# his0si/ConvNet-Quantization

Hardware: AMD Instinct MI355X
Metric: images/sec at batch 1024 (3×32×32) int8 static-PTQ, 1/2/4/8 MI355X; top-1 delta (higher is better)
Workload: dtype int8; 1 GPU; full static-PTQ SimpleConvNet, all conv+linear int8 (u8 x s8 -> i32), NHWC, per-tensor weights; global_batch=1024, per_gpu_batch=1024, parallelism=dp1

## Files before the change

### convnet-quantization_amd/csrc/conv3x3.hip

```cpp
#include "common.hpp"
#include "conv_epi.hpp"
#include "conv_launch.hpp"
#include <type_traits>
#include <utility>
#include <algorithm>
#include <cmath>
#include "qconvnet_abi.hpp"

namespace qcn {

constexpr int kPipeD = 2;
constexpr int kSm56D = 4;
constexpr int kProdPrio = 2;

template <int CIN, int COUT, int HW, bool POOL, int WPX, int PSP = 16, int RPAD = 0,
          int SPAD = 0, bool SPLIT = false, int WI_ = 2, int JT_ = 4, int RB_ = 0>
struct ConvCfg {
  static constexpr int kCin = CIN, kCout = COUT;
  static constexpr bool kPool = POOL, kSplit = SPLIT;
  static constexpr int W = HW, H = HW;
  static constexpr int WI = WI_;
  static constexpr int JT = JT_;
  static constexpr int MPS = JT * WI;
  static constexpr int kWpx = WPX;
// ... 1320 lines not shown
      return dst ? reinterpret_cast<float4*>(eka) + e : const_cast<float4*>(reinterpret_cast<const float4*>(s) + o);
    }
    e -= NA;
    if (e < NB) {
      const int a = e / (CB::kCout / 4), o = e % (CB::kCout / 4);
      const float* s = a == 0 ? epb.u : (a == 1 ? epb.v : epb.mult);
      return dst ? reinterpret_cast<float4*>(ekb) + e : const_cast<float4*>(reinterpret_cast<const float4*>(s) + o);
    }
    e -= NB;
    if (e < NCA)
      return dst ? reinterpret_cast<float4*>(cra) + e
                 : const_cast<float4*>(reinterpret_cast<const float4*>(epa.corr) + e);
    e -= NCA;
    return dst ? reinterpret_cast<float4*>(crb) + e
               : const_cast<float4*>(reinterpret_cast<const float4*>(epb.corr) + e);
  };
  {
    const uint32_t pa4 = xor80(splat_u8(x_zp)), pb4 = xor80(splat_u8(xb_zp));
    auto halo = [&](auto cfg, uint8_t* base, int nbuf, int pbytes, uint32_t pad) {
      using C = decltype(cfg);
      constexpr int HS = 2 * C::PCOLS + 2 * (C::PROWS - 2), CH = C::kCin / 16;
      const int total = nbuf * C::SEGS * HS * CH;
      for (int e = tid; e < total; e += 512) {
        const int c = e % CH, hs = (e / CH) % HS, sg = (e / (CH * HS)) % C::SEGS, bf = e / (CH * HS * C::SEGS);
        int pr, pc;
        if (hs < C::PCOLS) { pr = 0; pc = hs; }
        else if (hs < 2 * C::PCOLS) { pr = C::PROWS - 1; pc = hs - C::PCOLS; }
        else { const int r = hs - 2 * C::PCOLS; pr = 1 + (r >> 1); pc = (r & 1) ? C::PCOLS - 1 : 0; }
        *reinterpret_cast<uint4*>(base + bf * pbytes + C::slot(sg, pr, pc) + c * 16) = make_uint4(pad, pad, pad, pad);
      }
    };
    halo(CA{}, lds + P::OFF_PA, P::DOUBLE_A ? 2 : 1, P::PA, pa4);
    halo(CB{}, lds + P::OFF_PB, 2, P::PB, pb4);
  }
  if (role == 1) {
#pragma unroll
    for (int k = 0; k < TPT; ++k)
      if (rt + 256 * k < NTAB) tval[k] = *tab(rt + 256 * k, false);
#pragma unroll
    for (int k = 0; k < TPT; ++k)
      if (rt + 256 * k < NTAB) *tab(rt + 256 * k, true) = tval[k];
  }
  if (T == 0) return;

  const int p16 = lane & 15, g = lane >> 4;
  const wt_rsrc_t wra = wt_rsrc(wa), wrb = wt_rsrc(wb);
  const int voff = (wc * 64 + p16) * 64 + g * 16;
  auto pa_buf = [&](int j) { return lds + P::OFF_PA + (P::DOUBLE_A ? (j & 1) * P::PA : 0); };
  auto pb_buf = [&](int j) { return lds + P::OFF_PB + (j & 1) * P::PB; };
  auto write_in = [&](uint8_t* pa, const uint4 (&sv)[4]) {
#pragma unroll
    for (int q = 0; q < 4; ++q)
      *reinterpret_cast<uint4*>(pa + in_dst(q)) =
          make_uint4(xor80(sv[q].x), xor80(sv[q].y), xor80(sv[q].z), xor80(sv[q].w));
  };
  auto first_chunk = [&](wt_rsrc_t w0, v4i (&ga)[2][4]) {
#pragma unroll
    for (int i = 0; i < 4; ++i) {
      const auto v = __builtin_amdgcn_raw_buffer_load_b128(w0, voff, i * 1024, 0);
      ga[0][i] = (v4i){(int)v[0], (int)v[1], (int)v[2], (int)v[3]};
    }
  };

  v4i acc[4][8];
  if (role == 0) write_in(pa_buf(0), sv0);
  lds_barrier();

  struct Lane {
    int p16, g, ek;
    int la, lb;
    int hb;
    int q;
    const int *ca, *cb;
  };
  auto lanes = [&]() {
    int lz = lane;
    asm volatile("" : "+v"(lz));
    Lane L;
    L.p16 = lz & 15;
    L.g = lz >> 4;
    L.ek = wc * 64 + 4 * L.g;
    L.la = XA::at(wp, 0, L.p16) + 16 * L.g;
    L.lb = XB::at(wp, 0, L.p16) + 16 * L.g;
    L.hb = XA::template out_at<CB>(wp, 0, L.p16) + wc * 64 + 4 * L.g;
    L.q = wp * 32 + L.p16;
    L.ca = cra + (lz >> 6);
    L.cb = crb + (lz >> 6);
    return L;
  };
  auto epi_a = [&](const Lane& L, uint8_t* pb) {
    static_for<4>([&](auto ic) {
      constexpr int i = decltype(ic)::value;
      const EpiG K = load_epig(eka, CA::kCout, L.ek + 16 * i);
      static_for<8>([&](auto jc) {
        constexpr int j = decltype(jc)::value;
        uint32_t wd = 0;
#pragma unroll
        for (int r = 0; r < 4; ++r) wd = rq_elem<FA>(acc[i][j][r], K, r, epa, wd);
        *reinterpret_cast<uint32_t*>(pb + L.hb + XA::template out_jofs<CB>(j) + 16 * i) = xor80(wd);
      });
    });
  };
  auto epi_b = [&](const Lane& L, int k) {
    static_for<2>([&](auto gc) {
      constexpr int gq = decltype(gc)::value;
      uint32_t d[4];
      static_for<4>([&](auto ic) {
        constexpr int i = decltype(ic)::value;
        const EpiG K = load_epig(ekb, CB::kCout, L.ek + 16 * i);
        uint32_t wd = 0;
#pragma unroll
        for (int r = 0; r < 4; ++r) {
          const int a = max(max(acc[i][4 * gq][r], acc[i][4 * gq + 1][r]),
                            max(acc[i][4 * gq + 2][r], acc[i][4 * gq + 3][r]));
          wd = rq_elem<FB>(a, K, r, epb, wd);
        }
        d[i] = wd;
      });
      const auto s02 = __builtin_amdgcn_permlane32_swap(d[0], d[2], false, false);
      const auto s13 = __builtin_amdgcn_permlane32_swap(d[1], d[3], false, false);
      const auto t01 = __builtin_amdgcn_permlane16_swap(s02[0], s13[0], false, false);
      const auto t23 = __builtin_amdgcn_permlane16_swap(s02[1], s13[1], false, false);
      const uint4 v = make_uint4(t01[0], t01[1], t23[0], t23[1]);
      const int q = L.q + 16 * gq;
      const int n = img_of(k, q / P::OPI), pix = q % P::OPI;
      const int co = wc * 64 + 16 * L.g;
      const bool real = ILV ? b + (k * SEGS + q / P::OPI) * G < nimg : (b + k * G) * SEGS + q / P::OPI < nimg;
      if (real) {
        if constexpr (KMAJOR) {
          const int kc = (pix * CB::kCout + co) / 32;
          store_wt16(wt_rsrc(y), (uint32_t)(((long)kc * nimg + n) * 32 + 16 * (L.g & 1)), v);
        } else {
          store_wt16(wt_rsrc(y + (long)n * P::OPI * CB::kCout), (uint32_t)(pix * CB::kCout + co), v);
        }
      }
    });
  };

  if (role == 0) {
    v4i ga[2][4];
    first_chunk(wra, ga);
    uint4 sv[4] = {};
#pragma unroll 1
    for (int p = 0; p <= T; ++p) {
      if constexpr (!P::DOUBLE_A) {
        if (p >= 1 && p < T) write_in(pa_buf(p), sv);
        lds_barrier();
      }
      WS16_STAMP(p, 0);
      if (p < T) {
        const Lane L = lanes();
        pipe_job16<CA>(pa_buf(p), L.ca, wra, wra, voff, wc, L.la, L.g, acc, ga);
        WS16_STAMP(p, 1);
        const int kn = p + 1 < T ? p + 1 : p;
#pragma unroll
        for (int q = 0; q < 4; ++q) sv[q] = *reinterpret_cast<const uint4*>(in_src(kn, q));
        epi_a(L, pb_buf(p));
        if constexpr (P::DOUBLE_A) write_in(pa_buf(p + 1), sv);
        WS16_STAMP(p, 2);
      }
      lds_barrier();
    }
  } else {
    v4i ga[2][4];
    first_chunk(wrb, ga);
#pragma unroll 1
    for (int p = 0; p <= T; ++p) {
      if constexpr (!P::DOUBLE_A) lds_barrier();
      WS16_STAMP(p, 0);
      if (p >= 1) {
        const Lane L = lanes();
        if (p >= 2) epi_b(L, p - 2);
        WS16_STAMP(p, 1);
        pipe_job16<CB>(pb_buf(p - 1), L.cb, wrb, wrb, voff, wc, L.lb, L.g, acc, ga);
        WS16_STAMP(p, 2);
      }
      lds_barrier();
    }
    const Lane L = lanes();
    epi_b(L, T - 1);
#ifdef QCN_CONVNET_STAMP
    if (T + 1 < 8) { WS16_STAMP(T + 1, 0); }
#endif
  }
}

template <class CA, class CB, int FA, int FB, bool KMAJOR>
__global__ __launch_bounds__(512, 1)
void convpair_ws16_kernel(const uint8_t* __restrict__ x, int nimg, int x_zp, const int8_t* __restrict__ wa,
                          ConvEpi epa, int xb_zp, const int8_t* __restrict__ wb, ConvEpi epb,
                          uint8_t* __restrict__ y) {
  convpair_ws16_body<CA, CB, FA, FB, KMAJOR>((int)blockIdx.x, (int)gridDim.x, x, nimg, x_zp, wa, epa, xb_zp,
                                             wb, epb, y);
}

using W16A3 = ConvCfg<64, 128, 16, false, 2, 32, 0, 0, false>;
using W16B4 = ConvCfg<128, 128, 16, true, 2, 32, 64, 0, true>;
using W16A5 = ConvCfg<128, 256, 8, false, 1, 32, 192, 0, false>;
using W16B6 = ConvCfg<256, 256, 8, true, 1, 32, 0, 0, true>;

struct Conv1Cfg {
  static constexpr int H = 32, W = 32, R = 16, COUT = 64, NT = 256;
  static constexpr int PXB = R * W;
  static constexpr int PR = R + 2, PC = W + 2;
  static constexpr int PATCH = 3 * PR * PC;
  static constexpr int PATCH_AL = (PATCH + 15) / 16 * 16;
  static constexpr int KS = 32 + 16;
  static constexpr int LDS = PATCH_AL + PXB * KS;
};

template <int HW>
__global__ __launch_bounds__(256, 3)
void conv1_f32_kernel(const float* __restrict__ x, int nimg, float in_inv, int in_zp,
                      const int8_t* __restrict__ w1, ConvEpi ep, uint8_t* __restrict__ y,
                      uint8_t* __restrict__ qin_out) {
  constexpr int H = HW, W = HW;
  constexpr int R = (HW * HW >= 512) ? 512 / W : H;
  constexpr int SEGS = (HW * HW >= 512) ? 1 : 512 / (HW * HW);
  constexpr int PR = R + 2, PC = W + 2;
  constexpr int PATCH = SEGS * 3 * PR * PC;
  constexpr int PATCH_AL = (PATCH + 15) / 16 * 16;
  constexpr int KS = 48;
  extern __shared__ __attribute__((aligned(16))) uint8_t lds[];
  int8_t* patch = reinterpret_cast<int8_t*>(lds);
  uint8_t* cols = lds + PATCH_AL;

  const int tid = threadIdx.x, lane = tid & 63, wave = tid >> 6;
  const int l32 = lane & 31, hi = lane >> 5;
  const long p0 = (long)blockIdx.x * 512;
  const int n0 = (int)(p0 / (H * W));
  const int y0 = (int)((p0 % (H * W)) / W);
  const int8_t padv = (int8_t)(in_zp - 128);

  for (int it = tid; it < PATCH; it += 256) {
    const int seg = it / (3 * PR * PC);
    const int rem = it % (3 * PR * PC);
    const int c = rem / (PR * PC);
    const int rr = (rem / PC) % PR, cc = rem % PC;
    const int n = n0 + seg, yy = y0 + rr - 1, xx = cc - 1;
    int8_t v = padv;
    if (n < nimg && yy >= 0 && yy < H && xx >= 0 && xx < W) {
      const long gi = (((long)n * 3 + c) * H + yy) * W + xx;
      float t = x[gi] * in_inv;
      t = fminf(fmaxf(t, -1.0e9f), 1.0e9f);
      int q = (int)__builtin_rintf(t) + in_zp;
      q = q < 0 ? 0 : (q > 255 ? 255 : q);
      v = (int8_t)(q - 128);
      if (qin_out != nullptr && seg < SEGS && rr >= 1 && rr <= R && cc >= 1 && cc <= W)
        qin_out[(((long)n * H + yy) * W + xx) * 3 + c] = (uint8_t)q;
    }
    patch[it] = v;
  }
  __syncthreads();
  for (int pp = tid; pp < 512; pp += 256) {
    const int seg = pp / (R * W), yy = (pp / W) % R, xx = pp % W;
    uint32_t wds[8];
#pragma unroll
    for (int d = 0; d < 8; ++d) {
      uint32_t wv = 0;
#pragma unroll
      for (int bb = 0; bb < 4; ++bb) {
        const int k = d * 4 + bb;
        uint32_t byte = 0;
        if (k < 27) {
          const int tap = k / 3, c = k % 3, r = tap / 3, s = tap % 3;
          byte = (uint8_t)patch[((seg * 3 + c) * PR + yy + r) * PC + xx + s];
        }
        wv |= byte << (8 * bb);
      }
      wds[d] = wv;
    }
    uint4* dst = reinterpret_cast<uint4*>(cols + pp * KS);
    dst[0] = make_uint4(wds[0], wds[1], wds[2], wds[3]);
    dst[1] = make_uint4(wds[4], wds[5], wds[6], wds[7]);
  }
  __syncthreads();

  v4i a[2];
#pragma unroll
  for (int i = 0; i < 2; ++i)
    a[i] = *reinterpret_cast<const v4i*>(w1 + (i * 32 + l32) * 32 + hi * 16);
  v16i acc[2][4];
#pragma unroll
  for (int j = 0; j < 4; ++j) {
    const int m = (wave * 4 + j) * 32 + l32;
    const v4i b = *reinterpret_cast<const v4i*>(cols + m * KS + hi * 16);
#pragma unroll
    for (int i = 0; i < 2; ++i)
      acc[i][j] = __builtin_amdgcn_mfma_i32_32x32x32_i8(a[i], b, acc_init_corr(ep.corr, i * 32, hi),
                                                        0, 0, 0);
  }
  __syncthreads();
  uint8_t* lout = lds;
#pragma unroll
  for (int i = 0; i < 2; ++i)
#pragma unroll
    for (int j = 0; j < 4; ++j)
      epilogue_tile<1>(&acc[i][j], ep, i * 32, hi, lout + ((wave * 4 + j) * 32 + l32) * 80);
  __syncthreads();
  const long total = (long)nimg * H * W;
  store_staged<64, 80, 256>(lout, 512, y + p0 * 64, total - p0, tid);
}

using Conv2Cfg = ConvCfg<64, 64, 32, true, 4, 16, 96, 0, true>;

struct Conv12P {
  using C = Conv2Cfg;
  static constexpr int PATCH = C::PATCH;
  static constexpr int WRES = 9 * C::WBUF;
  static constexpr int IN_R = 20, IN_C = 40;
  static constexpr int IN8 = IN_R * IN_C * 4;
  static constexpr int OFF_W = 2 * PATCH;
  static constexpr int OFF_IN = OFF_W + WRES;
  static constexpr int OFF_EPI1 = OFF_IN + 2 * IN8;
  static constexpr int OFF_EPI2 = OFF_EPI1 + 12 * 64;
  static constexpr int OFF_CORR2 = OFF_EPI2 + 12 * 64;
  static constexpr int OFF_A1 = OFF_CORR2 + 4 * 64;
  static constexpr int OFF_CORR1 = OFF_A1 + 2 * 64 * 16;
  static constexpr int LDS = OFF_CORR1 + 4 * 64;
  static_assert(LDS <= 160 * 1024, "LDS budget");
  static constexpr int OFF_QLUT = LDS;
  static constexpr int LDS_U8 = OFF_QLUT + 3 * 256;
  static_assert(OFF_QLUT % 4 == 0 && LDS_U8 <= 160 * 1024, "LDS budget");
};

template <class C>
QCN_DEV void conv_mainloop_res(const uint8_t* patch, const uint8_t* wres,
                               const int* __restrict__ corr, int wave, int lane,
                               v16i (&acc)[2][4]) {
  constexpr int CB = C::kCin / 64;
  const int wc = wave % C::WCO, wp = wave / C::WCO;
  const int l32 = lane & 31, hi = lane >> 5;
  const PatchAddr<C> pa(wp, l32, hi);
  const int arow = wc * 64 + l32;
  const int aswz = (arow >> 2) & 3;
  v16i c0[2];
#pragma unroll
  for (int i = 0; i < 2; ++i) c0[i] = acc_init_corr(corr, wc * 64 + i * 32, hi);
  const uint8_t* abase = wres + arow * 64;
  auto rd_a = [&](int ch, int kk, int i) {
    return *reinterpret_cast<const v4i*>(abase + ch * C::WBUF + i * 32 * 64 +
                                         (((2 * kk + hi) ^ aswz) << 4));
  };
  auto rd_b = [&](int ch, int kk, int j) {
    const int tap = ch / CB, cb = ch % CB;
    return *reinterpret_cast<const v4i*>(patch + pa.base[j] + PatchAddr<C>::delta(tap, j) + cb * 64 +
                                         kk * 32);
  };
  auto step = [&](v4i (&fan)[2], v4i (&fbn)[4], int rch, int rkk, bool rd,
                  const v4i (&fa)[2], const v4i (&fb)[4], bool first) {
#pragma unroll
    for (int m = 0; m < 8; ++m) {
      if (rd) {
        if (m < 2) fan[m] = rd_a(rch, rkk, m);
        else if (m < 6) fbn[m - 2] = rd_b(rch, rkk, m - 2);
      }
      __builtin_amdgcn_sched_barrier(0);
      acc[m >> 2][m & 3] = __builtin_amdgcn_mfma_i32_32x32x32_i8(
          fa[m >> 2], fb[m & 3], first ? c0[m >> 2] : acc[m >> 2][m & 3], 0, 0, 0);
      __builtin_amdgcn_sched_barrier(0);
    }
  };
  v4i fa0[2], fb0[4], fa1[2], fb1[4];
  fa0[0] = rd_a(0, 0, 0);
  fa0[1] = rd_a(0, 0, 1);
#pragma unroll
  for (int j = 0; j < 4; ++j) fb0[j] = rd_b(0, 0, j);
#pragma unroll
  for (int ch = 0; ch < C::NCH; ++ch) {
    step(fa1, fb1, ch, 1, true, fa0, fb0, ch == 0);
    step(fa0, fb0, ch + 1, 0, ch + 1 < C::NCH, fa1, fb1, false);
  }
}

#ifdef QCN_C12_STAMP
__device__ unsigned long long g_c12_stamp[4096][3][12][3];
QCN_DEV void c12_stamp(int j, int k) {
  const unsigned long long t = __builtin_amdgcn_s_memtime();
  const unsigned lane = __builtin_amdgcn_mbcnt_hi(~0u, __builtin_amdgcn_mbcnt_lo(~0u, 0u));
  const int w = threadIdx.x >> 6;
  const int s = w == 0 ? 0 : (w == 4 ? 1 : (w == 5 ? 2 : -1));
  if (s >= 0 && lane == 0 && blockIdx.x < 4096 && j < 12) {
    volatile unsigned long long* d = &g_c12_stamp[blockIdx.x][s][j][k];
    *d = t + lane;
  }
}
#define C12_STAMP(j, k) c12_stamp(j, k)
#else
#define C12_STAMP(j, k)
#endif

template <class XT>
QCN_DEV void conv12p_body(int t0, int ts, int T, const XT* __restrict__ x, int nimg,
                          float in_inv, int in_zp, const int8_t* __restrict__ w1, ConvEpi ep1,
                          int x2_zp, const int8_t* __restrict__ w2, ConvEpi ep2,
                          uint8_t* __restrict__ y, const uint8_t* __restrict__ qlut = nullptr) {
  using C = Conv2Cfg;
  using L = Conv12P;
  constexpr bool U8 = std::is_same<XT, uint8_t>::value;
  static_assert(U8 || std::is_same<XT, float>::value, "fp32 NCHW or u8 NHWC input");
  extern __shared__ __attribute__((aligned(16))) uint8_t lds[];
  const int tid = threadIdx.x, lane = tid & 63, wave = tid >> 6;
  const bool producer = wave >= 4;
  const int ptid = tid - 320;
  auto tile_of = [&](int j) { return (t0 + (j >> 1) * ts) * 2 + (j & 1); };
  uint8_t* patch0 = lds;
  uint8_t* patch1 = lds + L::PATCH;
  uint8_t* in8_0 = lds + L::OFF_IN;
  uint8_t* in8_1 = lds + L::OFF_IN + L::IN8;

  typename std::conditional<U8, uint32_t, float4>::type xraw[3];
  const uint32_t padw = xor80(splat_u8(x2_zp));
  const uint4 pad4 = make_uint4(padw, padw, padw, padw);
  for (int e = tid; e < 2 * C::PROWS * 8; e += 512) {
    const int buf = e / (C::PROWS * 8), r = e % (C::PROWS * 8);
    const int pr = r / 8, pc = ((r / 4) & 1) ? C::PCOLS - 1 : 0, chunk = r & 3;
    *reinterpret_cast<uint4*>(lds + buf * L::PATCH + C::slot(0, pr, pc) + chunk * 16) = pad4;
  }

  auto setup = [&]() {
    if (!producer) {
      const int wave_u = __builtin_amdgcn_readfirstlane(wave);
#pragma unroll
      for (int i = 0; i < L::WRES / 4096; ++i) {
        const int p = i * 4 + wave_u;
        const int o = p * 1024 + lane * 16;
        const int ch = o / C::WBUF, oc = o % C::WBUF;
        const int r = oc >> 6, sl = (oc >> 4) & 3;
        glds16(w2 + (long)ch * C::WBUF + r * 64 + ((sl ^ ((r >> 2) & 3)) << 4), lds + L::OFF_W + p * 1024);
      }
    }

    const uint32_t in_pad = xor80(splat_u8(in_zp)) & 0x00ffffffu;
    for (int e = tid; e < 2 * L::IN_R * L::IN_C; e += 512) {
      const int b = e / (L::IN_R * L::IN_C), rc = e % (L::IN_R * L::IN_C);
      const int rr = rc / L::IN_C, cc = rc % L::IN_C;
      const bool pad_row = b == 0 ? rr < 2 : rr >= 18;
      if (pad_row || cc < 4 || cc >= 36)
        reinterpret_cast<uint32_t*>(lds + L::OFF_IN + b * L::IN8)[rc] = in_pad;
    }
    if (!producer) stage_epik<64, 256>(ep1, reinterpret_cast<float*>(lds + L::OFF_EPI1), tid);
    if (!producer) stage_epik<64, 256>(ep2, reinterpret_cast<float*>(lds + L::OFF_EPI2), tid);
    {
      int t = tid;
      asm volatile("" : "+v"(t));
      if (t < 16)
        reinterpret_cast<int4*>(lds + L::OFF_CORR2)[t] = reinterpret_cast<const int4*>(ep2.corr)[t];
      if (t >= 64 && t < 80)
        reinterpret_cast<int4*>(lds + L::OFF_CORR1)[t - 64] = reinterpret_cast<const int4*>(ep1.corr)[t - 64];
    }
    if (wave == 3) {
      const int l32 = lane & 31, hi = lane >> 5;
      v4i* a1t = reinterpret_cast<v4i*>(lds + L::OFF_A1);
#pragma unroll
      for (int i = 0; i < 2; ++i) {
        const uint4 r0 = *reinterpret_cast<const uint4*>(w1 + (i * 32 + l32) * 32);
        const uint4 r1 = *reinterpret_cast<const uint4*>(w1 + (i * 32 + l32) * 32 + 16);
        const uint32_t wd[8] = {r0.x, r0.y, r0.z, r0.w, r1.x, r1.y, r1.z, r1.w};
        auto byte = [&](int k) -> uint32_t { return (wd[k >> 2] >> (8 * (k & 3))) & 0xff; };
        auto tapw = [&](int t) -> int {
          return (int)(byte(3 * t) | (byte(3 * t + 1) << 8) | (byte(3 * t + 2) << 16));
        };
        const v4i lo4 = (v4i){tapw(0) | (int)(byte(24) << 24), tapw(1) | (int)(byte(25) << 24),
                              tapw(2) | (int)(byte(26) << 24), tapw(3)};
        const v4i hi4 = (v4i){tapw(4), tapw(5), tapw(6), tapw(7)};
        a1t[i * 64 + lane] = hi ? hi4 : lo4;
      }
    }
    if constexpr (U8) {
      for (int e = tid; e < 3 * 256; e += 512) lds[L::OFF_QLUT + e] = qlut[e] ^ 0x80;
    }
  };
  auto fresh_ptid = [&]() {
    int v = ptid;
    asm volatile("" : "+v"(v));
    return v;
  };
  auto stage_load = [&](int t) {
    if (ptid < 0) return;
    const int n = t >> 1, y0 = (t & 1) * 16;
    const int pt = fresh_ptid();
    const int r = pt < 144 ? pt >> 3 : 0, g = pt & 7;
    const int iy = y0 + (y0 == 0 ? 0 : -2) + r;
    const int nc = n < nimg ? n : nimg - 1;
    if constexpr (U8) {
      const uint32_t* p = reinterpret_cast<const uint32_t*>(x + (((long)nc * 32 + iy) * 32 + 4 * g) * 3);
#pragma unroll
      for (int c = 0; c < 3; ++c) xraw[c] = p[c];
    } else {
#pragma unroll
      for (int c = 0; c < 3; ++c)
        xraw[c] = *reinterpret_cast<const float4*>(x + (((long)nc * 3 + c) * 32 + iy) * 32 + 4 * g);
    }
  };
  auto stage_store = [&](uint8_t* in8, int half) {
    const int pt = fresh_ptid();
    if (pt >= 0 && pt < 144) {
      const int rr = (half ? 0 : 2) + (pt >> 3), g = pt & 7;
      uint32_t wd[4];
      if constexpr (U8) {
        const uint8_t* lut = lds + L::OFF_QLUT;
#pragma unroll
        for (int e = 0; e < 4; ++e) {
          uint32_t d = 0;
#pragma unroll
          for (int c = 0; c < 3; ++c) {
            const int k = 3 * e + c;
            const uint32_t b = (xraw[k >> 2] >> (8 * (k & 3))) & 0xffu;
            d |= (uint32_t)lut[c * 256 + b] << (8 * c);
          }
          wd[e] = d;
        }
      } else {
        const float zpf = (float)in_zp;
#pragma unroll
        for (int e = 0; e < 4; ++e) {
          uint32_t d = 0;
#pragma unroll
          for (int c = 0; c < 3; ++c) {
            const float xv = e == 0 ? xraw[c].x : e == 1 ? xraw[c].y : e == 2 ? xraw[c].z : xraw[c].w;
            d = __builtin_amdgcn_cvt_pk_u8_f32(__builtin_rintf(xv * in_inv) + zpf, c, d);
          }
          wd[e] = d ^ 0x00808080u;
        }
      }
      *reinterpret_cast<uint4*>(in8 + (rr * L::IN_C + 4 + 4 * g) * 4) = make_uint4(wd[0], wd[1], wd[2], wd[3]);
    }
  };
  auto fresh = [](int v) {
    asm volatile("" : "+v"(v));
    return v;
  };
  bool vuni = false, muni = false;
  const bool fast1 = epi_fast(ep1);
  auto conv1_tile = [&](int t, const uint8_t* in8, uint8_t* pb, const uint8_t* prev, int w,
                        int step) {
    __builtin_amdgcn_s_setprio(kProdPrio);
    const int h = t & 1, y0 = h * 16;
    const int r0 = h == 0 ? 1 : (prev ? 2 : 0), r1 = h == 0 ? 18 : 17;
    const int ln = fresh(lane), l32 = ln & 31, hi = ln >> 5;
    if (w == step - 1) {
      uint8_t* prow_ptr = pb + C::slot(0, h == 0 ? 0 : 17, l32 + 1);
      *reinterpret_cast<uint4*>(prow_ptr + hi * 32) = pad4;
      *reinterpret_cast<uint4*>(prow_ptr + hi * 32 + 16) = pad4;
    }
    if (prev) {
      for (int e = w * 64 + ln; e < 2 * C::RS / 16; e += step * 64)
        *reinterpret_cast<uint4*>(pb + C::slot(0, 0, 0) + e * 16) =
            *reinterpret_cast<const uint4*>(prev + C::slot(0, 16, 0) + e * 16);
    }
    const float* ek1 = reinterpret_cast<const float*>(lds + L::OFF_EPI1);
    v4i a1[2];
    v16i c1[2];
    {
      const v4i* a1t = reinterpret_cast<const v4i*>(lds + L::OFF_A1);
      const int* corr1 = reinterpret_cast<const int*>(lds + L::OFF_CORR1);
#pragma unroll
      for (int i = 0; i < 2; ++i) {
        a1[i] = a1t[i * 64 + ln];
        c1[i] = acc_init_corr(corr1, i * 32, hi);
      }
    }
    const int* in32 = reinterpret_cast<const int*>(in8);
    auto bop = [&](int tr, v4i& b0) {
      const int* r0 = in32 + (tr + 0) * L::IN_C + l32 + 3;
      const int* r1 = r0 + L::IN_C;
      const int* r2 = r1 + L::IN_C;
      if (hi == 0) {
        const uint32_t t8 = (uint32_t)r2[2];
        b0 = (v4i){(int)__builtin_amdgcn_perm((uint32_t)r0[0], t8, 0x00060504u),
                   (int)__builtin_amdgcn_perm((uint32_t)r0[1], t8, 0x01060504u),
                   (int)__builtin_amdgcn_perm((uint32_t)r0[2], t8, 0x02060504u), r1[0]};
      } else {
        b0 = (v4i){r1[1], r1[2], r2[0], r2[1]};
      }
    };
    auto rows = [&](auto mode) {
      constexpr int MODE = decltype(mode)::value > 2 ? decltype(mode)::value - 2 : decltype(mode)::value;
      constexpr bool AFF = decltype(mode)::value > 2;
      float u[2][16], m[2][16];
      const float sv = ek1[64], sm = ek1[128];
      if constexpr (MODE != 0) {
#pragma unroll
        for (int i = 0; i < 2; ++i)
#pragma unroll
          for (int g = 0; g < 4; ++g) {
            const int co = i * 32 + 8 * g + 4 * hi;
            const float4 u4 = *reinterpret_cast<const float4*>(ek1 + co);
            u[i][4 * g] = u4.x; u[i][4 * g + 1] = u4.y; u[i][4 * g + 2] = u4.z; u[i][4 * g + 3] = u4.w;
            if constexpr (MODE == 2) {
              const float4 m4 = *reinterpret_cast<const float4*>(ek1 + 128 + co);
              m[i][4 * g] = m4.x; m[i][4 * g + 1] = m4.y; m[i][4 * g + 2] = m4.z; m[i][4 * g + 3] = m4.w;
            }
          }
      }
      if constexpr (MODE == 0) {
        for (int tr = r0 + w; tr < r1; tr += step) {
          const int iy = y0 - 1 + tr;
          uint8_t* prow_ptr = pb + C::slot(0, tr, l32 + 1);
          if (iy < 0 || iy >= 32) {
            *reinterpret_cast<uint4*>(prow_ptr + hi * 32) = pad4;
            *reinterpret_cast<uint4*>(prow_ptr + hi * 32 + 16) = pad4;
            continue;
          }
          v4i b0;
          bop(tr, b0);
#pragma unroll
          for (int i = 0; i < 2; ++i) {
            v16i acc = __builtin_amdgcn_mfma_i32_32x32x32_i8(a1[i], b0, c1[i], 0, 0, 0);
            epilogue_tile_kf<1, true>(&acc, load_epik_lds(ek1, 64, i * 32, hi), ep1, i * 32, hi,
                                      prow_ptr);
          }
        }
      } else {
        const int wr = r0 + w;
        const int nr = (r1 - wr + step - 1) / step;
        auto mfma_row = [&](int tr, v16i (&acc)[2]) {
          v4i b0;
          bop(tr, b0);
#pragma unroll
          for (int i = 0; i < 2; ++i)
            acc[i] = __builtin_amdgcn_mfma_i32_32x32x32_i8(a1[i], b0, c1[i], 0, 0, 0);
        };
        auto requant_row = [&](const v16i (&acc)[2], int tr) {
          v2f t[2][8];
#pragma unroll
          for (int i = 0; i < 2; ++i)
#pragma unroll
            for (int e = 0; e < 16; ++e) {
              float f = (float)acc[i][e];
              f = __builtin_fmaf(u[i][e], sv, f);
              f = f * (MODE == 1 ? sm : m[i][e]);
              if constexpr (AFF) f = qdq_aff_f(f, ep1);
              t[i][e >> 1][e & 1] = f;
            }
          uint8_t* prow_ptr = pb + C::slot(0, tr, l32 + 1);
          uint32_t* pdw = reinterpret_cast<uint32_t*>(prow_ptr) + hi;
#pragma unroll
          for (int i = 0; i < 2; ++i)
#pragma unroll
            for (int g = 0; g < 4; ++g) {
              uint32_t wd = __builtin_amdgcn_cvt_pk_u8_f32(t[i][2 * g].x, 0, 0u);
              wd = __builtin_amdgcn_cvt_pk_u8_f32(t[i][2 * g].y, 1, wd);
              wd = __builtin_amdgcn_cvt_pk_u8_f32(t[i][2 * g + 1].x, 2, wd);
              wd = __builtin_amdgcn_cvt_pk_u8_f32(t[i][2 * g + 1].y, 3, wd);
              pdw[i * 8 + 2 * g] = xor80(wd);
            }
          const int iy = y0 - 1 + tr;
          if (iy < 0 || iy >= 32) {
            *reinterpret_cast<uint4*>(prow_ptr + hi * 32) = pad4;
            *reinterpret_cast<uint4*>(prow_ptr + hi * 32 + 16) = pad4;
          }
        };
        v16i acc_x[2], acc_y[2];
        if (nr > 0) mfma_row(wr, acc_x);
#pragma unroll
        for (int kr = 0; kr < 5; kr += 2) {
          if (kr >= nr) break;
          if (kr + 1 < nr) mfma_row(wr + step * (kr + 1), acc_y);
          requant_row(acc_x, wr + step * kr);
          if (kr + 1 < nr) {
            if (kr + 2 < nr) mfma_row(wr + step * (kr + 2), acc_x);
            requant_row(acc_y, wr + step * (kr + 1));
          }
        }
      }
    };
    if (fast1 && vuni) {
      if (muni) rows(std::integral_constant<int, 1>{});
      else rows(std::integral_constant<int, 2>{});
    } else if (ep1.qdq == 2 && vuni) {
      if (muni) rows(std::integral_constant<int, 3>{});
      else rows(std::integral_constant<int, 4>{});
    } else {
      rows(std::integral_constant<int, 0>{});
    }
  };
  auto conv2_tile = [&](int t, const uint8_t* pb) {
    const int ln = fresh(lane), l32 = ln & 31, hi = ln >> 5;
    v16i acc[2][4];
    conv_mainloop_res<C>(pb, lds + L::OFF_W, reinterpret_cast<const int*>(lds + L::OFF_CORR2),
                         wave, ln, acc);
    C12_STAMP(((t >> 1) - t0) / ts * 2 + (t & 1) + 1, 2);
    const int n = t >> 1, h = t & 1;
    const float* ek2 = reinterpret_cast<const float*>(lds + L::OFF_EPI2);
    uint8_t* dst = y + ((long)n * 256 + h * 128 + wave * 32 + l32) * 64;
    const uint8_t* wbase = y + ((long)n * 256 + h * 128) * 64;
    const uint32_t woff = (uint32_t)((wave * 32 + l32) * 64);
#pragma unroll
    for (int i = 0; i < 2; ++i)
      epilogue_tile_kf<4, false, false, true>(acc[i], load_epik_lds(ek2, 64, i * 32, hi), ep2, i * 32, hi,
                                              dst, wbase, woff);
  };

  if (producer && T > 0) stage_load(tile_of(0));
  setup();
  if constexpr (U8) __syncthreads();
  if (producer && T > 0) stage_store(in8_0, 0);
  if (!producer) asm volatile("s_waitcnt vmcnt(0)" ::: "memory");
  __syncthreads();
  {
    const float* ek1 = reinterpret_cast<const float*>(lds + L::OFF_EPI1);
    const int l = lane;
    vuni = __builtin_amdgcn_ballot_w64(ek1[64 + l] != ek1[64]) == 0;
    muni = __builtin_amdgcn_ballot_w64(ek1[128 + l] != ek1[128]) == 0;
  }
  constexpr bool SPLIT0 = true;
  for (int j = 0; j <= T; ++j) {
    C12_STAMP(j, 0);
    if (producer) {
      if (j + 1 < T) stage_load(tile_of(j + 1));
      if (j < T) {
        const bool split = SPLIT0 && j == 0;
        conv1_tile(tile_of(j), (j & 1) ? in8_1 : in8_0, (j & 1) ? patch1 : patch0,
                   (j & 1) ? patch0 : nullptr, split ? wave : wave - 4, split ? 8 : 4);
      }
      if (j + 1 < T) stage_store(((j + 1) & 1) ? in8_1 : in8_0, (j + 1) & 1);
    } else if (j >= 1) {
      conv2_tile(tile_of(j - 1), ((j - 1) & 1) ? patch1 : patch0);
    } else if (SPLIT0 && T > 0) {
      conv1_tile(tile_of(0), in8_0, patch0, nullptr, wave, 8);
      __builtin_amdgcn_s_setprio(0);
    }
    C12_STAMP(j, 1);
    __syncthreads();
  }
}

#ifndef QCN_CONV_U8_TU
__global__ __launch_bounds__(512, 1)
void conv12p_kernel(const float* __restrict__ x, int nimg, float in_inv, int in_zp,
                    const int8_t* __restrict__ w1, ConvEpi ep1, int x2_zp,
                    const int8_t* __restrict__ w2, ConvEpi ep2, uint8_t* __restrict__ y) {
  const int T = (int)blockIdx.x < nimg ? 2 * ((nimg - 1 - (int)blockIdx.x) / (int)gridDim.x + 1) : 0;
  conv12p_body((int)blockIdx.x, (int)gridDim.x, T, x, nimg, in_inv, in_zp, w1, ep1, x2_zp, w2, ep2, y);
}
#endif

#define QCN_C16_PARAMS                                                                                   \
  const int8_t* __restrict__ w0, ConvEpi e0, int z0, const int8_t* __restrict__ w1, ConvEpi e1, int z1, \
      const int8_t* __restrict__ w2, ConvEpi e2, int z2, const int8_t* __restrict__ w3, ConvEpi e3,      \
      int z3, const int8_t* __restrict__ w4, ConvEpi e4, int z4, const int8_t* __restrict__ w5,          \
      ConvEpi e5, int z5
#define QCN_C16_ARGS(L)                                                                                  \
  (L).w[0], (L).ep[0], (L).x_zp[0], (L).w[1], (L).ep[1], (L).x_zp[1], (L).w[2], (L).ep[2], (L).x_zp[2],   \
      (L).w[3], (L).ep[3], (L).x_zp[3], (L).w[4], (L).ep[4], (L).x_zp[4], (L).w[5], (L).ep[5], (L).x_zp[5]

struct ConvnetLayers {
  const int8_t* w[6];
  ConvEpi ep[6];
  int x_zp[6];
};

using SmA3 = ConvCfg<64, 128, 16, false, 4, 16, 96, 0, false, 2, 2>;
using SmB4 = ConvCfg<128, 128, 16, true, 2, 16, 32, 0, true, 1, 4>;
using SmA5 = ConvCfg<128, 256, 8, false, 1, 16, 224, 0, false, 1, 2>;
using SmB6 = ConvCfg<256, 256, 8, true, 1, 16, 32, 64, true, 1, 2>;

using WsA3 = ConvCfg<64, 128, 16, false, 2, 16, 96, 0, false>;
using WsB4 = ConvCfg<128, 128, 16, true, 2, 16, 32, 0, true>;
using WsA5 = ConvCfg<128, 256, 8, false, 1, 16, 224, 0, false>;
using WsB6 = ConvCfg<256, 256, 8, true, 1, 16, 32, 64, true>;

constexpr int cmax(int a, int b) { return a > b ? a : b; }
constexpr int kConvnet16Lds = cmax(Conv12P::LDS, cmax(PairWs16<W16A3, W16B4>::LDS, PairWs16<W16A5, W16B6>::LDS));
constexpr int kConvnetSmLds = cmax(Conv12P::LDS, cmax(PairCfg<SmA3, SmB4>::LDS, PairGaCfg<SmA5, SmB6>::LDS));

#ifdef QCN_CONVNET_STAMP
__device__ unsigned long long g_c16_stamp[4096][8];
QCN_DEV void c16_stamp(int i) {
  const unsigned long long t = __builtin_amdgcn_s_memtime();
  const unsigned long long r = __builtin_amdgcn_s_memrealtime();
  const unsigned lane = __builtin_amdgcn_mbcnt_hi(~0u, __builtin_amdgcn_mbcnt_lo(~0u, 0u));
  if ((threadIdx.x >> 6) == 0 && lane == 0 && blockIdx.x < 4096) {
    volatile unsigned long long* d = g_c16_stamp[blockIdx.x];
    d[i] = t + lane;
    d[4 + i] = r + lane;
  }
}
#define C16_STAMP(i) c16_stamp(i)
#else
#define C16_STAMP(i)
#endif

QCN_DEV void phase_boundary() {
  asm volatile("s_waitcnt vmcnt(0) lgkmcnt(0)" ::: "memory");
  __builtin_amdgcn_s_setprio(0);
  __syncthreads();
}

template <int EM, bool KMAJOR>
__global__ __launch_bounds__(512, 1)
void convnet_convs16_kernel(const float* __restrict__ x, int nimg, float in_inv, QCN_C16_PARAMS,
                            uint8_t* __restrict__ a2, uint8_t* __restrict__ a4, uint8_t* __restrict__ a6) {
  static_assert(PairWs16<W16A3, W16B4>::SEGS == 1, "conv3+4 tile k of workgroup b is image b + kG");
  const int b = (int)blockIdx.x, G = (int)gridDim.x;
  const int T = b < nimg ? 2 * ((nimg - 1 - b) / G + 1) : 0;
  C16_STAMP(0);
  conv12p_body(b, G, T, x, nimg, in_inv, z0, w0, e0, z1, w1, e1, a2);
  phase_boundary();
  C16_STAMP(1);
  convpair_ws16_body<W16A3, W16B4, EM, EM, false>(b, G, a2, nimg, z2, w2, e2, z3, w3, e3, a4);
  phase_boundary();
  C16_STAMP(2);
  convpair_ws16_body<W16A5, W16B6, EM, EM, KMAJOR, true>(b, G, a4, nimg, z4, w4, e4, z5, w5, e5, a6);
#ifdef QCN_CONVNET_STAMP
  __syncthreads();
#endif
  C16_STAMP(3);
}

#ifndef QCN_CONV_U8_TU
__global__ __launch_bounds__(512, 1)
void convnet_convs_sm_kernel(const float* __restrict__ x, int nimg, float in_inv, QCN_C16_PARAMS,
                             uint8_t* __restrict__ a2, uint8_t* __restrict__ a4, uint8_t* __restrict__ a6) {
  const int b = (int)blockIdx.x;
  C16_STAMP(0);
  conv12p_body(b, (int)gridDim.x, 2, x, nimg, in_inv, z0, w0, e0, z1, w1, e1, a2);
  phase_boundary();
  C16_STAMP(1);
  convpair_body<SmA3, SmB4>(b, a2, nimg, z2, w2, e2, z3, w3, e3, a4);
  phase_boundary();
  C16_STAMP(2);
  convpair_ga_body<SmA5, SmB6, kSm56D>(b, a4, nimg, z4, w4, e4, z5, w5, e5, a6);
#ifdef QCN_CONVNET_STAMP
  __syncthreads();
#endif
  C16_STAMP(3);
}

struct ConvsF32 {
  static constexpr auto sm = convnet_convs_sm_kernel;
  template <int EM, bool KMAJOR>
  static constexpr auto k16 = convnet_convs16_kernel<EM, KMAJOR>;
  static constexpr int kLdsSm = kConvnetSmLds, kLds16 = kConvnet16Lds;
};
#endif

int convnet_convs_plan(int nimg, float in_scale, int in_zp, const qcn_conv_layer_t* layers, int kmajor,
                       ConvnetLayers& L, int& em, int& ncu);


template <auto K, int LDS, class X, class IN>
int conv12_fused(const X* x, int nimg, IN in, const qcn_conv_layer_t& l1, const qcn_conv_layer_t& l2, uint8_t* y,
                 void* stream) {
  if (!x || !y || nimg <= 0 || !layer_ok(l1) || !layer_ok(l2)) return QCN_ERR_ARG;
  const ConvEpi ep1 = make_epi(l1), ep2 = make_epi(l2);
  const int ncu = qcn_cu_count();
  if (ncu <= 0) return QCN_ERR_HIP;
  return launch_lds<K>(dim3(nimg < ncu ? nimg : ncu), dim3(512), LDS, (hipStream_t)stream, x, nimg, in,
                       l1.x_zp, l1.w, ep1, l2.x_zp, l2.w, ep2, y);
}

template <class F, class X, class IN>
int convnet_convs(const X* x, int nimg, IN in, float in_scale, int in_zp, const qcn_conv_layer_t* layers,
                  uint8_t* a2, uint8_t* a4, uint8_t* a6, int kmajor, void* stream) {
  if (!x || !layers || !a2 || !a4 || !a6) return QCN_ERR_ARG;
  ConvnetLayers L;
  int em = 0, ncu = 0;
  const int form = convnet_convs_plan(nimg, in_scale, in_zp, layers, kmajor, L, em, ncu);
  if (form < 0) return form;
  hipStream_t st = (hipStream_t)stream;
  if (form == 1)
    return launch_lds<F::sm>(dim3(nimg), dim3(512), F::kLdsSm, st, x, nimg, in, QCN_C16_ARGS(L), a2, a4, a6);
#define QCN_C16(EM_, KM_)                                                                                \
  if (em == EM_ && (kmajor != 0) == KM_)                                                                 \
    return launch_lds<F::template k16<EM_, KM_>>(dim3(ncu), dim3(512), F::kLds16, st, x, nimg, in,       \
                                                 QCN_C16_ARGS(L), a2, a4, a6);
  QCN_C16(1, true) QCN_C16(1, false) QCN_C16(2, true) QCN_C16(2, false)
#undef QCN_C16
  return QCN_ERR_UNSUPPORTED;
}

#ifndef QCN_CONV_U8_TU
__global__ void conv3x3_generic_kernel(const uint8_t* __restrict__ x, int nimg, int H, int W,
                                       int cin, int x_zp, const int8_t* __restrict__ wpk,
                                       int tiled, int cout, ConvEpi ep, int pool,
                                       uint8_t* __restrict__ y) {
  const int OH = pool ? H / 2 : H, OW = pool ? W / 2 : W;
  const long total = (long)nimg * OH * OW * cout;
  for (long e = blockIdx.x * (long)blockDim.x + threadIdx.x; e < total;
       e += (long)gridDim.x * blockDim.x) {
    const int co = (int)(e % cout);
    const long pix = e / cout;
    const int ox = (int)(pix % OW), oy = (int)((pix / OW) % OH);
    const int n = (int)(pix / ((long)OW * OH));
    int best = INT32_MIN;
    const int nq = pool ? 4 : 1;
    for (int qd = 0; qd < nq; ++qd) {
      const int yy = pool ? 2 * oy + (qd >> 1) : oy;
      const int xx = pool ? 2 * ox + (qd & 1) : ox;
      int acc = 0;
      for (int r = 0; r < 3; ++r)
        for (int s = 0; s < 3; ++s) {
          const int iy = yy + r - 1, ix = xx + s - 1;
          if (iy < 0 || iy >= H || ix < 0 || ix >= W) continue;
          const uint8_t* xp = x + (((long)n * H + iy) * W + ix) * cin;
          const int tap = r * 3 + s;
          for (int c = 0; c < cin; ++c) {
            const long wi = tiled ? ((long)(tap * (cin / 64) + c / 64) * cout + co) * 64 + (c % 64)
                                  : ((long)co * 9 + tap) * cin + c;
            acc += ((int)xp[c] - x_zp) * (int)wpk[wi];
          }
        }
      best = acc > best ? acc : best;
    }
    int q = requant_one(best, ep.u[co], ep.v[co], ep.mult[co], ep.zp_y, ep.lo);
    if (ep.qdq) q = qdq_next(q, ep.s1, ep.z1, ep.inv2, ep.z2);
    y[e] = (uint8_t)q;
  }
}

namespace {

float qdq_ref_host(float q1, const ConvEpi& ep) {
  float x = (q1 - (float)ep.z1) * ep.s1;
  x = x > 0.0f ? x : 0.0f;
  const float t = std::fmin(x * ep.inv2, 1.0e9f);
  const float r = std::nearbyint(t) + (float)ep.z2;
  return std::fmin(std::fmax(r, 0.0f), 255.0f);
}

float rne_sat_u8(float x) {
  const float r = std::nearbyint(x);
  return std::fmin(std::fmax(r, 0.0f), 255.0f);
}

bool qdq_affine_solve(ConvEpi& ep) {
  const int zp = ep.zp_y, lo = ep.lo;
  const int r0 = lo - zp, r1 = 255 - zp;
  if (r0 > r1) return false;
  auto g = [&](int r) {
    const float q1 = std::fmin(std::fmax((float)r + (float)zp, (float)lo), 255.0f);
    return qdq_ref_host(q1, ep);
  };
  const float glo = g(r0), ghi = g(r1);
  const double c = (double)ep.s1 * (double)ep.inv2;
  if (!(c > 0.0) || !std::isfinite(c)) return false;
  for (int k = 0; k < 81; ++k) {
    const double d = ((k + 1) / 2) * 1.0e-7 * ((k & 1) ? -1.0 : 1.0);
    const float qa = (float)(c * (1.0 + d));
    if (!(qa > 0.0f)) continue;
    double lb = -1.0e30, ub = 1.0e30;
    for (int r = r0; r <= r1; ++r) {
      const double gr = g(r), ar = (double)qa * r;
      if (gr > glo) lb = std::max(lb, gr - 0.5 - ar);
      if (gr < ghi) ub = std::min(ub, gr + 0.5 - ar);
    }
    double mid;
    if (lb > -1.0e29 && ub < 1.0e29) mid = 0.5 * (lb + ub);
    else if (lb > -1.0e29) mid = lb + 0.25;
    else if (ub < 1.0e29) mid = ub - 0.25;
    else mid = (double)glo;
    if (!(lb < ub)) continue;
    const float qb = (float)mid;
    bool ok = true;
    for (int r = r0; r <= r1 && ok; ++r) {
      const float v = std::fmin(std::fmax(std::fma((float)r, qa, qb), glo), ghi);
      ok = rne_sat_u8(v) == g(r);
    }
    if (ok) {
      ep.qa = qa; ep.qb = qb; ep.glo = glo; ep.ghi = ghi;
      return true;
    }
  }
  return false;
}

}

void set_qdq(ConvEpi& ep, const qcn_qdq_t* q) {
  ep.qdq = 1;
  ep.s1 = q->s1; ep.z1 = q->z1; ep.inv2 = q->inv2; ep.z2 = q->z2;
  struct Entry { float s1, inv2; int z1, z2, zp, lo; bool ok; float qa, qb, glo, ghi; };
  static thread_local Entry cache[16];
  static thread_local int ncache = 0, next = 0;
  for (int i = 0; i < ncache; ++i) {
    const Entry& e = cache[i];
    if (e.s1 == ep.s1 && e.inv2 == ep.inv2 && e.z1 == ep.z1 && e.z2 == ep.z2 && e.zp == ep.zp_y &&
        e.lo == ep.lo) {
      if (e.ok) { ep.qdq = 2; ep.qa = e.qa; ep.qb = e.qb; ep.glo = e.glo; ep.ghi = e.ghi; }
      return;
    }
  }
  const bool ok = qdq_affine_solve(ep);
  if (ok) ep.qdq = 2;
  cache[next] = Entry{ep.s1, ep.inv2, ep.z1, ep.z2, ep.zp_y, ep.lo, ok, ep.qa, ep.qb, ep.glo, ep.ghi};
  next = (next + 1) % 16;
  if (ncache < 16) ++ncache;
}
#endif

}

#ifndef QCN_NO_ABI
#include "qconvnet_abi.hpp"

namespace {
using namespace qcn;

template <class C>
int pixel_grid(int nimg) {
  return (int)(((long)nimg * C::IMG + C::PXB - 1) / C::PXB);
}

template <int CIN, int COUT, int HW, bool POOL, int WPX, int PSP = 16, int RPAD = 0,
          int SPAD = 0, bool SPLIT = false, int JT = 4, int RB = 0>
int launch_conv(const uint8_t* x, int nimg, int x_zp, const int8_t* wpk, const ConvEpi& ep,
                uint8_t* y, hipStream_t st) {
  using C = ConvCfg<CIN, COUT, HW, POOL, WPX, PSP, RPAD, SPAD, SPLIT, 2, JT, RB>;
  return launch_lds<conv3x3_u8s8_kernel<CIN, COUT, HW, POOL, WPX, PSP, RPAD, SPAD, SPLIT, JT, RB>>(
      dim3(pixel_grid<C>(nimg)), dim3(C::NT), C::LDS, st, x, nimg, x_zp, wpk, ep, y);
}

struct PairArgs {
  const uint8_t* x;
  int nimg, x_zp;
  const int8_t* wa;
  ConvEpi epa;
  int xb_zp;
  const int8_t* wb;
  ConvEpi epb;
  uint8_t* y;
};
// ... 308 lines not shown
```

Before: 7.972 million images/sec.

## Switch fused conv2 mainloop to 16x16x64 MFMA with shared overlapping patch rows

Rewrites the fused conv1->conv2 kernel's conv2 mainloop to use 16x16x64 int8 MFMA tiles, with each wave covering all output channels for 32 pixels and a new LDS swizzle for the resident weights. The two patch buffers now overlap in one row-shared region, and pad rows are written once at setup instead of in every tile. The pooled epilogue is redone with in-register max and permlane swaps feeding wide stores. This aims to cut LDS traffic and per-tile padding work and to improve MFMA efficiency, at the cost of more accumulator registers and more intricate buffer aliasing.

```diff
diff --git a/convnet-quantization_amd/csrc/conv3x3.hip b/convnet-quantization_amd/csrc/conv3x3.hip
--- a/convnet-quantization_amd/csrc/conv3x3.hip
+++ b/convnet-quantization_amd/csrc/conv3x3.hip
@@ -1646,15 +1646,19 @@
   store_staged<64, 80, 256>(lout, 512, y + p0 * 64, total - p0, tid);
 }
 
-using Conv2Cfg = ConvCfg<64, 64, 32, true, 4, 16, 96, 0, true>;
+using Conv2Cfg = ConvCfg<64, 64, 32, true, 4, 32, 0, 0, true>;
 
 struct Conv12P {
   using C = Conv2Cfg;
-  static constexpr int PATCH = C::PATCH;
+  static constexpr int ROWS = 2 * C::PROWS - 1;
+  static constexpr int OFF_BOT = 0;
+  static constexpr int OFF_TOP = (C::PROWS - 1) * C::RS;
+  static constexpr int PAD_ROW = C::PROWS - 1;
+  static constexpr int PATCHES = ROWS * C::RS;
   static constexpr int WRES = 9 * C::WBUF;
   static constexpr int IN_R = 20, IN_C = 40;
   static constexpr int IN8 = IN_R * IN_C * 4;
-  static constexpr int OFF_W = 2 * PATCH;
+  static constexpr int OFF_W = PATCHES;
   static constexpr int OFF_IN = OFF_W + WRES;
   static constexpr int OFF_EPI1 = OFF_IN + 2 * IN8;
   static constexpr int OFF_EPI2 = OFF_EPI1 + 12 * 64;
@@ -1668,53 +1672,52 @@
   static_assert(OFF_QLUT % 4 == 0 && LDS_U8 <= 160 * 1024, "LDS budget");
 };
 
+QCN_DEV constexpr int res16_swz(int r) { return (4 - ((r >> 2) & 3)) & 3; }
+
 template <class C>
-QCN_DEV void conv_mainloop_res(const uint8_t* patch, const uint8_t* wres,
-                               const int* __restrict__ corr, int wave, int lane,
-                               v16i (&acc)[2][4]) {
-  constexpr int CB = C::kCin / 64;
-  const int wc = wave % C::WCO, wp = wave / C::WCO;
-  const int l32 = lane & 31, hi = lane >> 5;
-  const PatchAddr<C> pa(wp, l32, hi);
-  const int arow = wc * 64 + l32;
-  const int aswz = (arow >> 2) & 3;
-  v16i c0[2];
-#pragma unroll
-  for (int i = 0; i < 2; ++i) c0[i] = acc_init_corr(corr, wc * 64 + i * 32, hi);
-  const uint8_t* abase = wres + arow * 64;
-  auto rd_a = [&](int ch, int kk, int i) {
-    return *reinterpret_cast<const v4i*>(abase + ch * C::WBUF + i * 32 * 64 +
-                                         (((2 * kk + hi) ^ aswz) << 4));
-  };
-  auto rd_b = [&](int ch, int kk, int j) {
-    const int tap = ch / CB, cb = ch % CB;
-    return *reinterpret_cast<const v4i*>(patch + pa.base[j] + PatchAddr<C>::delta(tap, j) + cb * 64 +
-                                         kk * 32);
-  };
-  auto step = [&](v4i (&fan)[2], v4i (&fbn)[4], int rch, int rkk, bool rd,
-                  const v4i (&fa)[2], const v4i (&fb)[4], bool first) {
-#pragma unroll
-    for (int m = 0; m < 8; ++m) {
-      if (rd) {
-        if (m < 2) fan[m] = rd_a(rch, rkk, m);
-        else if (m < 6) fbn[m - 2] = rd_b(rch, rkk, m - 2);
-      }
+QCN_DEV void conv_mainloop_res16(const uint8_t* patch, const uint8_t* wres, const int* corr, int wp,
+                                 int p16, int g, v4i (&acc)[4][8]) {
+  using X = Pix16<C>;
+  constexpr int S = C::NCH;
+  static_assert(X::affine(), "pixel blocks at constant offsets");
+  static_assert(C::kCin == 64 && C::kCout == 64 && C::WCO == 1, "one tap per K-step, all couts per wave");
+  const int lb = X::at(wp, 0, p16) + 16 * g;
+  const int la = p16 * 64 + ((g ^ res16_swz(p16)) << 4);
+  v4i c0[4];
+#pragma unroll
+  for (int i = 0; i < 4; ++i) c0[i] = *reinterpret_cast<const v4i*>(corr + 16 * i + 4 * g);
+  auto rd_a = [&](int s, int i) {
+    return *reinterpret_cast<const v4i*>(wres + la + s * C::WBUF + i * 1024);
+  };
+  auto rd_b = [&](int s, int j) {
+    return *reinterpret_cast<const v4i*>(patch + lb + X::jofs(j) + PatchAddr<C>::delta(s, j));
+  };
+  v4i fa[2][4], fb[8];
+#pragma unroll
+  for (int i = 0; i < 4; ++i) fa[0][i] = rd_a(0, i);
+#pragma unroll
+  for (int j = 0; j < 8; ++j) fb[j] = rd_b(0, j);
+  static_for<S>([&](auto sc) {
+    constexpr int s = decltype(sc)::value;
+    static_for<32>([&](auto mc) {
+      constexpr int m = decltype(mc)::value, j = s == 0 ? (m & 7) : (m >> 2), i = s == 0 ? (m >> 3) : (m & 3);
       __builtin_amdgcn_sched_barrier(0);
-      acc[m >> 2][m & 3] = __builtin_amdgcn_mfma_i32_32x32x32_i8(
-          fa[m >> 2], fb[m & 3], first ? c0[m >> 2] : acc[m >> 2][m & 3], 0, 0, 0);
+      acc[i][j] = __builtin_amdgcn_mfma_i32_16x16x64_i8(fa[s & 1][i], fb[j], s == 0 ? c0[i] : acc[i][j], 0, 0, 0);
       __builtin_amdgcn_sched_barrier(0);
-    }
-  };
-  v4i fa0[2], fb0[4], fa1[2], fb1[4];
-  fa0[0] = rd_a(0, 0, 0);
-  fa0[1] = rd_a(0, 0, 1);
-#pragma unroll
-  for (int j = 0; j < 4; ++j) fb0[j] = rd_b(0, 0, j);
-#pragma unroll
-  for (int ch = 0; ch < C::NCH; ++ch) {
-    step(fa1, fb1, ch, 1, true, fa0, fb0, ch == 0);
-    step(fa0, fb0, ch + 1, 0, ch + 1 < C::NCH, fa1, fb1, false);
-  }
+      if constexpr ((m & 3) == 1 && m < 16 && s + 1 < S) {
+        fa[(s + 1) & 1][m >> 2] = rd_a(s + 1, m >> 2);
+        __builtin_amdgcn_sched_barrier(0);
+      }
+      if constexpr (i == 3 && s + 1 < S) {
+        fb[j] = rd_b(s + 1, j);
+        __builtin_amdgcn_sched_barrier(0);
+      }
+    });
+#pragma unroll
+    for (int i = 0; i < 4; ++i)
+#pragma unroll
+      for (int j = 0; j < 8; ++j) asm volatile("" : "+v"(acc[i][j]));
+  });
 }
 
 #ifdef QCN_C12_STAMP
@@ -1746,20 +1749,34 @@
   extern __shared__ __attribute__((aligned(16))) uint8_t lds[];
   const int tid = threadIdx.x, lane = tid & 63, wave = tid >> 6;
   const bool producer = wave >= 4;
-  const int ptid = tid - 320;
   auto tile_of = [&](int j) { return (t0 + (j >> 1) * ts) * 2 + (j & 1); };
-  uint8_t* patch0 = lds;
-  uint8_t* patch1 = lds + L::PATCH;
+  uint8_t* patch0 = lds + L::OFF_TOP;
+  uint8_t* patch1 = lds + L::OFF_BOT;
   uint8_t* in8_0 = lds + L::OFF_IN;
   uint8_t* in8_1 = lds + L::OFF_IN + L::IN8;
 
-  typename std::conditional<U8, uint32_t, float4>::type xraw[3];
+  using XRaw = typename std::conditional<U8, uint32_t, float4>::type;
+  auto def_xraw = [](XRaw (&xr)[3]) {
+#pragma unroll
+    for (int c = 0; c < 3; ++c) {
+      if constexpr (U8) asm volatile("" : "=v"(xr[c]));
+      else asm volatile("" : "=v"(xr[c].x), "=v"(xr[c].y), "=v"(xr[c].z), "=v"(xr[c].w));
+    }
+  };
+  auto fresh_epi = [](const ConvEpi& ep) {
+    ConvEpi e = ep;
+    asm volatile("" : "+s"(e.zp_y), "+s"(e.lo), "+s"(e.z1), "+s"(e.z2));
+    return e;
+  };
   const uint32_t padw = xor80(splat_u8(x2_zp));
   const uint4 pad4 = make_uint4(padw, padw, padw, padw);
-  for (int e = tid; e < 2 * C::PROWS * 8; e += 512) {
-    const int buf = e / (C::PROWS * 8), r = e % (C::PROWS * 8);
-    const int pr = r / 8, pc = ((r / 4) & 1) ? C::PCOLS - 1 : 0, chunk = r & 3;
-    *reinterpret_cast<uint4*>(lds + buf * L::PATCH + C::slot(0, pr, pc) + chunk * 16) = pad4;
+  int th = tid;
+  asm volatile("" : "+v"(th));
+  for (int e = th; e < (2 * L::ROWS + C::PCOLS) * 4; e += 512) {
+    const int s = e >> 2, chunk = e & 3;
+    const int pr = s < 2 * L::ROWS ? s >> 1 : L::PAD_ROW;
+    const int pc = s < 2 * L::ROWS ? ((s & 1) ? C::PCOLS - 1 : 0) : s - 2 * L::ROWS;
+    *reinterpret_cast<uint4*>(lds + L::OFF_BOT + C::slot(0, pr, pc) + chunk * 16) = pad4;
   }
 
   auto setup = [&]() {
@@ -1771,7 +1788,7 @@
         const int o = p * 1024 + lane * 16;
         const int ch = o / C::WBUF, oc = o % C::WBUF;
         const int r = oc >> 6, sl = (oc >> 4) & 3;
-        glds16(w2 + (long)ch * C::WBUF + r * 64 + ((sl ^ ((r >> 2) & 3)) << 4), lds + L::OFF_W + p * 1024);
+        glds16(w2 + (long)ch * C::WBUF + r * 64 + ((sl ^ res16_swz(r)) << 4), lds + L::OFF_W + p * 1024);
       }
     }
 
@@ -1816,14 +1833,14 @@
     }
   };
   auto fresh_ptid = [&]() {
-    int v = ptid;
+    int v = tid;
     asm volatile("" : "+v"(v));
-    return v;
-  };
-  auto stage_load = [&](int t) {
-    if (ptid < 0) return;
+    return v - 320;
+  };
+  auto stage_load = [&](int t, XRaw (&xraw)[3]) {
+    const int pt = fresh_ptid();
+    if (pt < 0) return;
     const int n = t >> 1, y0 = (t & 1) * 16;
-    const int pt = fresh_ptid();
     const int r = pt < 144 ? pt >> 3 : 0, g = pt & 7;
     const int iy = y0 + (y0 == 0 ? 0 : -2) + r;
     const int nc = n < nimg ? n : nimg - 1;
@@ -1837,7 +1854,7 @@
         xraw[c] = *reinterpret_cast<const float4*>(x + (((long)nc * 3 + c) * 32 + iy) * 32 + 4 * g);
     }
   };
-  auto stage_store = [&](uint8_t* in8, int half) {
+  auto stage_store = [&](uint8_t* in8, int half, const XRaw (&xraw)[3]) {
     const int pt = fresh_ptid();
     if (pt >= 0 && pt < 144) {
       const int rr = (half ? 0 : 2) + (pt >> 3), g = pt & 7;
@@ -1875,19 +1892,15 @@
     asm volatile("" : "+v"(v));
     return v;
   };
+  auto wave_s = [&]() { return __builtin_amdgcn_readfirstlane(fresh(tid) >> 6); };
   bool vuni = false, muni = false;
   const bool fast1 = epi_fast(ep1);
   auto conv1_tile = [&](int t, const uint8_t* in8, uint8_t* pb, const uint8_t* prev, int w,
                         int step) {
     __builtin_amdgcn_s_setprio(kProdPrio);
-    const int h = t & 1, y0 = h * 16;
+    const int h = t & 1;
     const int r0 = h == 0 ? 1 : (prev ? 2 : 0), r1 = h == 0 ? 18 : 17;
-    const int ln = fresh(lane), l32 = ln & 31, hi = ln >> 5;
-    if (w == step - 1) {
-      uint8_t* prow_ptr = pb + C::slot(0, h == 0 ? 0 : 17, l32 + 1);
-      *reinterpret_cast<uint4*>(prow_ptr + hi * 32) = pad4;
-      *reinterpret_cast<uint4*>(prow_ptr + hi * 32 + 16) = pad4;
-    }
+    const int ln = fresh(tid) & 63, l32 = ln & 31, hi = ln >> 5;
     if (prev) {
       for (int e = w * 64 + ln; e < 2 * C::RS / 16; e += step * 64)
         *reinterpret_cast<uint4*>(pb + C::slot(0, 0, 0) + e * 16) =
@@ -1939,20 +1952,15 @@
           }
       }
       if constexpr (MODE == 0) {
+        const ConvEpi e1 = fresh_epi(ep1);
         for (int tr = r0 + w; tr < r1; tr += step) {
-          const int iy = y0 - 1 + tr;
           uint8_t* prow_ptr = pb + C::slot(0, tr, l32 + 1);
-          if (iy < 0 || iy >= 32) {
-            *reinterpret_cast<uint4*>(prow_ptr + hi * 32) = pad4;
-            *reinterpret_cast<uint4*>(prow_ptr + hi * 32 + 16) = pad4;
-            continue;
-          }
           v4i b0;
           bop(tr, b0);
 #pragma unroll
           for (int i = 0; i < 2; ++i) {
             v16i acc = __builtin_amdgcn_mfma_i32_32x32x32_i8(a1[i], b0, c1[i], 0, 0, 0);
-            epilogue_tile_kf<1, true>(&acc, load_epik_lds(ek1, 64, i * 32, hi), ep1, i * 32, hi,
+            epilogue_tile_kf<1, true>(&acc, load_epik_lds(ek1, 64, i * 32, hi), e1, i * 32, hi,
                                       prow_ptr);
           }
         }
@@ -1990,11 +1998,6 @@
               wd = __builtin_amdgcn_cvt_pk_u8_f32(t[i][2 * g + 1].y, 3, wd);
               pdw[i * 8 + 2 * g] = xor80(wd);
             }
-          const int iy = y0 - 1 + tr;
-          if (iy < 0 || iy >= 32) {
-            *reinterpret_cast<uint4*>(prow_ptr + hi * 32) = pad4;
-            *reinterpret_cast<uint4*>(prow_ptr + hi * 32 + 16) = pad4;
-          }
         };
         v16i acc_x[2], acc_y[2];
         if (nr > 0) mfma_row(wr, acc_x);
@@ -2021,26 +2024,54 @@
     }
   };
   auto conv2_tile = [&](int t, const uint8_t* pb) {
-    const int ln = fresh(lane), l32 = ln & 31, hi = ln >> 5;
-    v16i acc[2][4];
-    conv_mainloop_res<C>(pb, lds + L::OFF_W, reinterpret_cast<const int*>(lds + L::OFF_CORR2),
-                         wave, ln, acc);
+    const int ln = fresh(tid) & 63, p16 = ln & 15, g = ln >> 4;
+    const int wv = wave_s();
+    v4i acc[4][8];
+    conv_mainloop_res16<C>(pb, lds + L::OFF_W, reinterpret_cast<const int*>(lds + L::OFF_CORR2), wv, p16, g,
+                           acc);
     C12_STAMP(((t >> 1) - t0) / ts * 2 + (t & 1) + 1, 2);
     const int n = t >> 1, h = t & 1;
     const float* ek2 = reinterpret_cast<const float*>(lds + L::OFF_EPI2);
-    uint8_t* dst = y + ((long)n * 256 + h * 128 + wave * 32 + l32) * 64;
-    const uint8_t* wbase = y + ((long)n * 256 + h * 128) * 64;
-    const uint32_t woff = (uint32_t)((wave * 32 + l32) * 64);
-#pragma unroll
-    for (int i = 0; i < 2; ++i)
-      epilogue_tile_kf<4, false, false, true>(acc[i], load_epik_lds(ek2, 64, i * 32, hi), ep2, i * 32, hi,
-                                              dst, wbase, woff);
-  };
-
-  if (producer && T > 0) stage_load(tile_of(0));
-  setup();
-  if constexpr (U8) __syncthreads();
-  if (producer && T > 0) stage_store(in8_0, 0);
+    const ConvEpi e2 = fresh_epi(ep2);
+    const wt_rsrc_t wr = wt_rsrc(y + ((long)n * 256 + h * 128 + wv * 32) * 64);
+    auto epi = [&](auto mode) {
+      constexpr int EM = decltype(mode)::value;
+      static_for<2>([&](auto gc) {
+        constexpr int gq = decltype(gc)::value;
+        uint32_t d[4];
+        static_for<4>([&](auto ic) {
+          constexpr int i = decltype(ic)::value;
+          const EpiG K = load_epig(ek2, 64, 16 * i + 4 * g);
+          uint32_t wd = 0;
+#pragma unroll
+          for (int r = 0; r < 4; ++r) {
+            const int a = max(max(acc[i][4 * gq][r], acc[i][4 * gq + 1][r]),
+                              max(acc[i][4 * gq + 2][r], acc[i][4 * gq + 3][r]));
+            wd = rq_elem<EM>(a, K, r, e2, wd);
+          }
+          d[i] = wd;
+        });
+        const auto s02 = __builtin_amdgcn_permlane32_swap(d[0], d[2], false, false);
+        const auto s13 = __builtin_amdgcn_permlane32_swap(d[1], d[3], false, false);
+        const auto t01 = __builtin_amdgcn_permlane16_swap(s02[0], s13[0], false, false);
+        const auto t23 = __builtin_amdgcn_permlane16_swap(s02[1], s13[1], false, false);
+        store_wt16(wr, (uint32_t)((16 * gq + p16) * 64 + 16 * g),
+                   make_uint4(t01[0], t01[1], t23[0], t23[1]));
+      });
+    };
+    if (epi_fast(e2)) epi(std::integral_constant<int, 1>{});
+    else if (e2.qdq == 2) epi(std::integral_constant<int, 2>{});
+    else epi(std::integral_constant<int, 0>{});
+  };
+
+  {
+    XRaw xraw[3];
+    def_xraw(xraw);
+    if (producer && T > 0) stage_load(tile_of(0), xraw);
+    setup();
+    if constexpr (U8) __syncthreads();
+    if (producer && T > 0) stage_store(in8_0, 0, xraw);
+  }
   if (!producer) asm volatile("s_waitcnt vmcnt(0)" ::: "memory");
   __syncthreads();
   {
@@ -2053,17 +2084,20 @@
   for (int j = 0; j <= T; ++j) {
     C12_STAMP(j, 0);
     if (producer) {
-      if (j + 1 < T) stage_load(tile_of(j + 1));
+      XRaw xraw[3];
+      def_xraw(xraw);
+      if (j + 1 < T) stage_load(tile_of(j + 1), xraw);
       if (j < T) {
         const bool split = SPLIT0 && j == 0;
+        const int wv = wave_s();
         conv1_tile(tile_of(j), (j & 1) ? in8_1 : in8_0, (j & 1) ? patch1 : patch0,
-                   (j & 1) ? patch0 : nullptr, split ? wave : wave - 4, split ? 8 : 4);
-      }
-      if (j + 1 < T) stage_store(((j + 1) & 1) ? in8_1 : in8_0, (j + 1) & 1);
+                   (j & 1) ? patch0 : nullptr, split ? wv : wv - 4, split ? 8 : 4);
+      }
+      if (j + 1 < T) stage_store(((j + 1) & 1) ? in8_1 : in8_0, (j + 1) & 1, xraw);
     } else if (j >= 1) {
       conv2_tile(tile_of(j - 1), ((j - 1) & 1) ? patch1 : patch0);
     } else if (SPLIT0 && T > 0) {
-      conv1_tile(tile_of(0), in8_0, patch0, nullptr, wave, 8);
+      conv1_tile(tile_of(0), in8_0, patch0, nullptr, wave_s(), 8);
       __builtin_amdgcn_s_setprio(0);
     }
     C12_STAMP(j, 1);
```

After: 8.072 million images/sec (median of 6 runs). 1.01x the previous value.
